# theopaid/Parallel-Image-Convolution-using-MPI-OPENMP-and-CUDA

Measured on AMD Instinct MI355X. Metric: Mpixels/sec (and wall-time) for 1920x2520 RGB, 40 reps at 1/2/4/8 MI355X, higher is better.
Workload: dtype fp32-exact (packed 16-bit integer, bit-identical to the reference float32)

## Files before the change

parallel-image-convolution-using-mpi-openmp-and-cuda_amd/csrc/include/pconv/engine.hpp:

```cpp
#pragma once

#include <hip/hip_runtime_api.h>

#include <functional>
#include <map>
#include <memory>
#include <tuple>
#include <vector>

#include "pconv/device.hpp"
#include "pconv/filter.hpp"
#include "pconv/image.hpp"
#include "pconv/kernels.hpp"
#include "pconv/partition.hpp"
#include "pconv/schedule.hpp"

namespace pconv {

class BandEngine;

class HaloTransport {
 public:
  virtual ~HaloTransport() = default;
  virtual void exchange(BandEngine& e, int64_t depth, hipStream_t stream) = 0;
  virtual const char* name() const = 0;
  virtual bool capturable() const { return false; }
};

struct EngineOptions {
  int device = 0;
  int halo_depth = 1;
  int fuse = 1;
  bool overlap = true;
  bool use_graph = false;
  bool capture_exchanges = false;
  KernelVariant variant = KernelVariant::Auto;
  Border border = Border::Zero;
  hipStream_t compute_stream = nullptr;
  hipStream_t comm_stream = nullptr;
  bool timing = true;
  bool kernel_copies = false;
  int stream_chunks = 0;
  std::vector<int> stream_weights;
  int64_t stream_min_bytes = int64_t(8) << 20;
  bool cu_mask_queues = true;
  bool head_on_slot_streams = true;
  bool head_alt_uploads = true;
  bool lazy_head = true;
};

struct RunStats {
  double loop_ms = 0;
  double wall_ms = 0;
  int launches = 0;
  int exchanges = 0;
  int64_t image_launches = 0;
};

class BandEngine {
 public:
  BandEngine(const ImageGeom& geom, const Band& band, const Filter& filter, const EngineOptions& opt);
  ~BandEngine();

  const ImageGeom& geom() const { return geom_; }
  const Band& band() const { return band_; }
  const Filter& filter() const { return filter_; }
  const FrameLayout& layout() const { return lay_; }
  const EngineOptions& options() const { return opt_; }
  static constexpr size_t kMaxCachedGraphs = 64;
  size_t cached_graphs() const { return graphs_.size() + step_graphs_.size(); }
  size_t cached_step_graphs() const { return step_graphs_.size(); }
  hipStream_t compute_stream() const { return cs_; }
  hipStream_t comm_stream() const { return ms_; }

  void set_transport(std::shared_ptr<HaloTransport> t) { transport_ = std::move(t); }

  uint8_t* src_frame() const { return frame_[cur_].data() + lay_.offset(0); }
  uint8_t* dst_frame() const { return frame_[cur_ ^ 1].data() + lay_.offset(0); }
  uint8_t* frame_at(int which) const { return frame_[which & 1].data() + lay_.offset(0); }
  uint8_t* frame_base(int which) const { return frame_[which & 1].data(); }
  int cur() const { return cur_; }
  void set_cur(int c) { cur_ = c & 1; }

  void upload_rows(const uint8_t* host, int64_t host_pitch, int64_t r_begin, int64_t r_end,
                   hipStream_t stream = nullptr);
  void upload_rows_device(const uint8_t* dev, int64_t dev_pitch, int64_t r_begin, int64_t r_end);
  void set_halo_valid(bool v) { halo_valid_ = v; }
  bool input_preloaded(int64_t in_r0, int64_t in_r1) const;
  void download_rows(uint8_t* host, int64_t host_pitch, int64_t r_begin, int64_t r_end,
                     hipStream_t stream = nullptr);
  void download_rows_device(uint8_t* dev, int64_t dev_pitch, int64_t r_begin, int64_t r_end);

  void wait_stream(hipStream_t s);
  void signal_stream(hipStream_t s);

  void exchange_now(hipStream_t stream = nullptr);
  bool has_transport() const { return transport_ != nullptr; }

  void run(int reps);
  uint64_t residual();
  StableStats run_until_stable(int max_reps, int check_every,
// ... 35 lines not shown
  DeviceBuffer frame_[2];
  int cur_ = 0;
  bool halo_valid_ = false;
  int pre_exchanges_ = 0;
  DeviceBuffer res_count_;
  PinnedBuffer res_host_;
  Event res_ev_;
  uint64_t res_seen_ = 0;
  Stream own_cs_, own_ms_;
  hipStream_t cs_ = nullptr, ms_ = nullptr;
  Event ev_ready_, ev_halo_, ev_t0_, ev_t1_, ev_sync_;
  std::vector<Event> up_evs_, dn_evs_;
  bool stream_trace_ = false;
  std::vector<Event> st_ev_;
  size_t st_chunks_ = 0;
 public:
  void set_stream_trace(bool on) { stream_trace_ = on; }
  std::vector<std::vector<double>> stream_trace();
  std::vector<double> time_residual(int launches);
  void reserve_stream_events(size_t chunks) {
    while (up_evs_.size() < chunks) up_evs_.push_back(Event::create());
    while (dn_evs_.size() < chunks + 1) dn_evs_.push_back(Event::create());
  }

 private:
  std::shared_ptr<HaloTransport> transport_;
  RunStats stats_;
  double wall_t0_ = 0;
  bool timing_pending_ = false;
  std::map<std::pair<int, int>, hipGraphExec_t> graphs_;
  struct StepGraph {
    hipGraphExec_t exec = nullptr;
    int end_cur = 0;
    int launches = 0;
    int exchanges = 0;
  };
  void trim_graph_caches();
  std::map<std::tuple<int, int, const uint8_t*, int64_t, int64_t, uint8_t*>, StepGraph> step_graphs_;
};

class BandPipeline {
 public:
  BandPipeline(const ImageGeom& geom, const Band& band, const Filter& filter, const EngineOptions& opt, int slots,
               int concurrent = -1, bool slot_streams = false, bool step_graphs = true, bool slot_comm = false);
  ~BandPipeline();
  int slots() const { return static_cast<int>(slots_.size()); }
  BandEngine& slot(int i) { return *slots_.at(i); }
  void set_transport(std::shared_ptr<HaloTransport> t);
  void set_slot_transport(int k, std::shared_ptr<HaloTransport> t);
  void submit(const uint8_t* host_in, int64_t in_r0, int64_t in_r1, uint8_t* host_out, int reps);
  void drain();
  int64_t submitted() const { return count_; }
  int64_t streamed_heads() const { return streamed_heads_; }
  bool concurrent() const { return concurrent_; }
  bool graphs() const { return graphs_; }
  bool step_graphs() const { return graphs_ && step_graphs_; }
  void enable_trace(int images);
  std::vector<std::vector<double>> trace();
  void enable_marks(int images);
  std::vector<std::vector<double>> marks();
  bool ready(int k);
  void wait_image(int k);

 private:
  void trace_mark(int stage, hipStream_t s);
  void completion_mark(int k, bool before, bool streamed);
  void submit_image(int k, const uint8_t* host_in, int64_t in_r0, int64_t in_r1, uint8_t* host_out, int reps);
  struct HeldImage {
    const uint8_t* in = nullptr;
    int64_t r0 = 0, r1 = 0;
    uint8_t* out = nullptr;
    int reps = 0;
    bool valid = false;
  };
  HeldImage held_;
  bool force_graph_ = false;
  void issue_held(bool streamed);
  Stream h2d_, d2h_, comm_;
  std::vector<Stream> computes_;
  std::vector<Stream> slot_comms_;
  bool concurrent_ = false;
  bool graphs_ = false;
  bool step_graphs_ = true;
  std::vector<std::unique_ptr<BandEngine>> slots_;
  std::vector<Event> ev_up_, ev_done_, ev_free_, ev_halo_;
  int64_t burst_pos_ = 0;
  int64_t streamed_heads_ = 0;
  bool head_streaming_ = false;
  bool head_on_slots_ = false;
  Event ev_head_, h2d_wait_;
  std::vector<bool> used_;
  int64_t count_ = 0;
  std::vector<Event> trace_ev_;
  std::vector<int> trace_slot_;
  int64_t trace_first_ = 0;
  std::vector<Event> done_;
  Event burst_start_;
  std::vector<Event> mark_ev_;
  std::vector<std::pair<int, bool>> mark_info_;
  int64_t mark_first_ = 0;
};

class LocalCluster {
 public:
  LocalCluster(const ImageGeom& geom, int bands, const Filter& filter, const EngineOptions& opt);
  int size() const { return static_cast<int>(engines_.size()); }
  BandEngine& engine(int i) { return *engines_.at(i); }
  void upload(const uint8_t* host, bool preload_halo);
  void run(int reps, bool device_async = false);
  void download(uint8_t* host);
  void synchronize();

 private:
  ImageGeom geom_;
  std::vector<std::unique_ptr<BandEngine>> engines_;
  std::vector<Event> ev_phase_;
};

class NullTransport : public HaloTransport {
 public:
  void exchange(BandEngine&, int64_t, hipStream_t) override {}
  const char* name() const override { return "null (timing only)"; }
  bool capturable() const override { return true; }
};

class LocalTransport : public HaloTransport {
 public:
  explicit LocalTransport(std::vector<BandEngine*> peers) : peers_(std::move(peers)) {}
  void exchange(BandEngine& e, int64_t depth, hipStream_t stream) override;
  const char* name() const override { return "local-d2d"; }
  bool capturable() const override { return false; }

 private:
  std::vector<BandEngine*> peers_;
};

}
// ... 1 lines not shown
```

parallel-image-convolution-using-mpi-openmp-and-cuda_amd/csrc/include/pconv/schedule.hpp:

```cpp
#pragma once

#include <cstdint>
#include <string>
#include <vector>

#include "pconv/partition.hpp"

namespace pconv {

struct LaunchSpec {
  int steps = 1;
  int64_t lo = 0, hi = 0;
  bool after_halo = false;
};

struct Phase {
  int64_t exchange_depth = 0;
  int steps = 1;
  std::vector<LaunchSpec> launches;
};

struct PlanConfig {
  int halo_depth = 1;
  int fuse = 1;
  bool overlap = true;
  bool halo_preloaded = false;
};

std::vector<Phase> plan_band(const Band& band, int reps, const PlanConfig& cfg);

std::string describe_plan(const std::vector<Phase>& plan);

struct StreamChunk {
  int64_t up_lo = 0, up_hi = 0;
  std::vector<LaunchSpec> launches;
  std::vector<int> levels;
  int64_t down_lo = 0, down_hi = 0;
};

struct StreamPlan {
  int levels = 0;
  std::vector<StreamChunk> chunks;
};

bool streamable(const std::vector<Phase>& plan);

std::vector<int64_t> stream_cuts(int64_t in_lo, int64_t in_hi, int chunks);
std::vector<int64_t> stream_cuts_weighted(int64_t in_lo, int64_t in_hi, const std::vector<int>& weights);

StreamPlan plan_streamed(const std::vector<Phase>& plan, int64_t in_lo, int64_t in_hi, int64_t owned_rows,
                         const std::vector<int64_t>& cuts);

PlanConfig normalize_plan_config(PlanConfig cfg, int64_t min_band_rows, int max_fuse);

}
```

parallel-image-convolution-using-mpi-openmp-and-cuda_amd/csrc/src/engine.cpp:

```cpp
#include "pconv/engine.hpp"

#include <cstring>

#include "pconv/trace.hpp"

#include <algorithm>
#include <atomic>
#include <cstdlib>
#include <thread>

namespace pconv {

namespace {

PlanConfig engine_plan_config(const ImageGeom& geom, const Band& band, const Filter& f, const EngineOptions& opt) {
  PlanConfig c;
  c.fuse = supports_fusion(f, opt.variant) ? opt.fuse : 1;
  c.halo_depth = opt.halo_depth;
  c.overlap = opt.overlap;
  const int64_t min_rows = band.world > 1 ? geom.height / band.world : 0;
  return normalize_plan_config(c, min_rows, kMaxFusedSteps);
}

}
// ... 616 lines not shown
    }
    if (step_graphs && opt.stream_chunks > 1) {
      head_on_slots_ = opt.head_on_slot_streams && slots >= 3;
      if (!head_on_slots_) {
        h2d_ = Stream::create(0);
        d2h_ = Stream::create(0);
      }
      ev_head_ = Event::create();
      h2d_wait_ = Event::create();
      head_streaming_ = true;
      const size_t nchunks = std::max(static_cast<size_t>(std::max(opt.stream_chunks, 0)), opt.stream_weights.size());
      for (auto& e : slots_) e->reserve_stream_events(nchunks + 1);
      const int64_t rb = slots_[0]->layout().row_bytes;
      PinnedBuffer row(static_cast<size_t>(rb));
      std::memset(row.data(), 0, row.size());
      for (auto& e : slots_) {
        e->upload_rows(row.data(), rb, 0, 1, e->compute_stream());
        e->download_rows(row.data(), rb, 0, 1, e->compute_stream());
      }
      for (auto& e : slots_) e->synchronize();
    }
    used_.assign(slots, false);
    for (int i = 0; i < slots; ++i) done_.push_back(Event::create(true));
    burst_start_ = Event::create(true);
    return;
  }
  const bool nb = band.up >= 0 || band.down >= 0;
  int hw_queues = 4;
  if (const char* q = std::getenv("GPU_MAX_HW_QUEUES")) hw_queues = std::max(1, std::atoi(q));
  const int fixed = 2 + (nb ? 1 : 0);
  concurrent_ = concurrent < 0 ? (slots > 1 && hw_queues >= fixed + slots) : (concurrent > 0 && slots > 1);
  h2d_ = Stream::create(0);
  d2h_ = Stream::create(0);
  EngineOptions o = opt;
  o.use_graph = false;
  o.timing = false;
  if (nb) {
    comm_ = Stream::create(-1);
    o.comm_stream = comm_.get();
  }
  for (int i = 0; i < (concurrent_ ? slots : 1); ++i) computes_.push_back(Stream::create(0));
  for (int i = 0; i < slots; ++i) {
    o.compute_stream = computes_[concurrent_ ? i : 0].get();
    slots_.push_back(std::make_unique<BandEngine>(geom, band, filter, o));
    ev_up_.push_back(Event::create());
    ev_done_.push_back(Event::create());
    ev_free_.push_back(Event::create());
    ev_halo_.push_back(Event::create());
  }
  used_.assign(slots, false);
}

BandPipeline::~BandPipeline() {
  if (h2d_.get()) (void)hipStreamSynchronize(h2d_.get());
  for (auto& c : computes_) (void)hipStreamSynchronize(c.get());
  for (auto& c : slot_comms_) (void)hipStreamSynchronize(c.get());
  if (d2h_.get()) (void)hipStreamSynchronize(d2h_.get());
  if (comm_.get()) (void)hipStreamSynchronize(comm_.get());
}

void BandPipeline::set_slot_transport(int k, std::shared_ptr<HaloTransport> t) {
  PCONV_CHECK(graphs_, "per-slot transports need the slot-stream pipeline");
  slots_.at(k)->set_transport(std::move(t));
}

void BandPipeline::set_transport(std::shared_ptr<HaloTransport> t) {
  for (auto& s : slots_) s->set_transport(t);
}

void BandPipeline::submit(const uint8_t* host_in, int64_t in_r0, int64_t in_r1, uint8_t* host_out, int reps) {
  TraceRange tr("pconv.pipeline.submit");
  if (held_.valid) issue_held(false);
  const int k = static_cast<int>(count_ % static_cast<int64_t>(slots_.size()));
  if (graphs_ && step_graphs_ && head_streaming_ && burst_pos_ == 0 && slots_[0]->options().lazy_head) {
    burst_start_.record(slots_[static_cast<size_t>(k)]->compute_stream());
    completion_mark(k, true, false);
    held_ = HeldImage{host_in, in_r0, in_r1, host_out, reps, true};
    return;
  }
  if (graphs_ && burst_pos_ == 0) burst_start_.record(slots_[static_cast<size_t>(k)]->compute_stream());
  completion_mark(k, true, false);
  const int64_t heads = streamed_heads_;
  submit_image(k, host_in, in_r0, in_r1, host_out, reps);
  completion_mark(k, false, streamed_heads_ != heads);
  if (graphs_) done_[static_cast<size_t>(k)].record(slots_[static_cast<size_t>(k)]->compute_stream());
}

void BandPipeline::issue_held(bool streamed) {
  const HeldImage h = held_;
  held_.valid = false;
  const int k = static_cast<int>(count_ % static_cast<int64_t>(slots_.size()));
  const int64_t heads = streamed_heads_;
  force_graph_ = !streamed;
  submit_image(k, h.in, h.r0, h.r1, h.out, h.reps);
  force_graph_ = false;
  completion_mark(k, false, streamed_heads_ != heads);
  done_[static_cast<size_t>(k)].record(slots_[static_cast<size_t>(k)]->compute_stream());
}

bool BandPipeline::ready(int k) {
  if (held_.valid) issue_held(true);
  const hipError_t e = hipEventQuery(done_.at(static_cast<size_t>(k)).get());
  if (e == hipErrorNotReady) return false;
  PCONV_HIP_CHECK(e);
  return true;
}

void BandPipeline::wait_image(int k) {
  if (held_.valid) issue_held(true);
  done_.at(static_cast<size_t>(k)).sync();
}

void BandPipeline::completion_mark(int k, bool before, bool streamed) {
  if (mark_ev_.empty()) return;
  const int64_t i = count_ - mark_first_ - (before ? 0 : 1);
  if (i < 0 || i + 1 >= static_cast<int64_t>(mark_ev_.size())) return;
  if (before && i != 0) return;
  hipStream_t s = graphs_ ? slots_[static_cast<size_t>(k)]->compute_stream() : (before ? h2d_.get() : d2h_.get());
  if (before) {
    mark_ev_[0].record(s);
    return;
  }
  mark_ev_[static_cast<size_t>(i + 1)].record(s);
  mark_info_.emplace_back(k, streamed);
}

void BandPipeline::enable_marks(int images) {
  PCONV_CHECK(images >= 0, "mark capacity must be >= 0");
  mark_ev_.clear();
  mark_info_.clear();
  if (images == 0) return;
  for (int i = 0; i <= images; ++i) mark_ev_.push_back(Event::create(true));
  mark_first_ = count_;
}

std::vector<std::vector<double>> BandPipeline::marks() {
  drain();
  std::vector<std::vector<double>> out;
  for (size_t i = 0; i < mark_info_.size(); ++i)
    out.push_back({static_cast<double>(mark_info_[i].first), Event::elapsed_ms(mark_ev_[0], mark_ev_[i + 1]),
                   mark_info_[i].second ? 1.0 : 0.0});
  mark_ev_.clear();
  mark_info_.clear();
  return out;
}

void BandPipeline::submit_image(int k, const uint8_t* host_in, int64_t in_r0, int64_t in_r1, uint8_t* host_out,
                                int reps) {
  BandEngine& e = *slots_[static_cast<size_t>(k)];
  if (graphs_ && !step_graphs_) {
    const bool preloaded = e.input_preloaded(in_r0, in_r1);
    hipStream_t cs = e.compute_stream();
    trace_mark(0, cs);
    e.upload_rows(host_in, e.layout().row_bytes, in_r0, in_r1);
    trace_mark(1, cs);
    if (!preloaded && e.exchange_free(reps, true)) {
      e.exchange_now(cs);
    } else {
      e.set_halo_valid(preloaded);
    }
    e.run(reps);
    trace_mark(2, cs);
    e.download_rows(host_out, e.layout().row_bytes, 0, e.band().rows);
    trace_mark(3, cs);
    used_[k] = true;
    ++count_;
    return;
  }
  if (graphs_) {
    PCONV_CHECK(trace_ev_.empty(), "pipeline trace needs directly issued images (graph capture off)");
    const int64_t in_bytes = (in_r1 - in_r0) * e.layout().row_bytes;
    if (burst_pos_ == 0 && head_streaming_ && !force_graph_ && in_bytes >= e.options().stream_min_bytes) {
      const StreamPlan sp = e.stream_plan(reps, in_r0, in_r1);
      if (!sp.chunks.empty()) {
        e.set_cur(0);
        const int n = slots();
        hipStream_t up = head_on_slots_ ? computes_[static_cast<size_t>((k + 1) % n)].get() : h2d_.get();
        hipStream_t down = head_on_slots_ ? computes_[static_cast<size_t>((k + n - 1) % n)].get() : d2h_.get();
        hipStream_t up2 = head_on_slots_ && n >= 4 && e.options().head_alt_uploads
                              ? computes_[static_cast<size_t>((k + 2) % n)].get()
                              : nullptr;
        h2d_wait_.record(e.compute_stream());
        h2d_wait_.wait_on(up);
        if (up2) h2d_wait_.wait_on(up2);
        hipStream_t done = e.enqueue_streamed(host_in, in_r0, in_r1, host_out, sp, up, down, up2);
        if (done != e.compute_stream()) {
          ev_head_.record(done);
          ev_head_.wait_on(e.compute_stream());
        }
        ++burst_pos_;
        used_[k] = true;
        ++count_;
        ++streamed_heads_;
        return;
      }
    }
    e.process_graph(host_in, in_r0, in_r1, host_out, reps);
    ++burst_pos_;
    used_[k] = true;
    ++count_;
    return;
  }
  const bool preloaded = e.input_preloaded(in_r0, in_r1);
  if (used_[k]) ev_free_[k].wait_on(h2d_.get());
  if (e.options().stream_chunks > 1 && trace_ev_.empty()) {
    const StreamPlan sp = e.stream_plan(reps, in_r0, in_r1);
    if (!sp.chunks.empty()) {
      hipStream_t done = e.enqueue_streamed(host_in, in_r0, in_r1, host_out, sp, h2d_.get(), d2h_.get());
      ev_free_[k].record(done);
      used_[k] = true;
      ++count_;
      return;
    }
  }
  trace_mark(0, h2d_.get());
  e.upload_rows(host_in, e.layout().row_bytes, in_r0, in_r1, h2d_.get());
  trace_mark(1, h2d_.get());
  ev_up_[k].record(h2d_.get());
  e.set_halo_valid(preloaded);
  if (!preloaded && comm_.get() && e.has_transport() && reps > 0) {
    ev_up_[k].wait_on(comm_.get());
    e.exchange_now(comm_.get());
    ev_halo_[k].record(comm_.get());
    ev_halo_[k].wait_on(e.compute_stream());
  } else {
// ... 139 lines not shown
```

parallel-image-convolution-using-mpi-openmp-and-cuda_amd/csrc/src/py_module.cpp:

```cpp
#include <omp.h>
#include <pybind11/pybind11.h>
#include <pybind11/stl.h>

#include <cstring>

#include "pconv/app.hpp"
#include "pconv/batch_engine.hpp"
#include "pconv/cpu_stencil.hpp"
#include "pconv/device.hpp"
#include "pconv/engine.hpp"
#include "pconv/ipc_halo.hpp"
#include "pconv/kernels.hpp"
#include "pconv/partition.hpp"
#include "pconv/selftest.hpp"
#include "pconv/raw_io.hpp"
#include "pconv/rccl_comm.hpp"
#include "pconv/schedule.hpp"
#include "../kernels/swar.hpp"

namespace py = pybind11;
using namespace pconv;

namespace {

// ... 94 lines not shown
      });
  m.def("row_band", &row_band, py::arg("height"), py::arg("world"), py::arg("rank"));
  m.def("row_bands", &row_bands, py::arg("height"), py::arg("world"));
  m.def("reference_rows_division", &reference_rows_division);

  py::class_<LaunchSpec>(m, "LaunchSpec")
      .def_readonly("steps", &LaunchSpec::steps)
      .def_readonly("lo", &LaunchSpec::lo)
      .def_readonly("hi", &LaunchSpec::hi)
      .def_readonly("after_halo", &LaunchSpec::after_halo);
  py::class_<Phase>(m, "Phase")
      .def_readonly("exchange_depth", &Phase::exchange_depth)
      .def_readonly("steps", &Phase::steps)
      .def_readonly("launches", &Phase::launches);
  m.def(
      "plan_band",
      [](const Band& b, int reps, int halo_depth, int fuse, bool overlap, bool halo_preloaded) {
        PlanConfig c;
        c.halo_depth = halo_depth;
        c.fuse = fuse;
        c.overlap = overlap;
        c.halo_preloaded = halo_preloaded;
        return plan_band(b, reps, c);
      },
      py::arg("band"), py::arg("reps"), py::arg("halo_depth") = 1, py::arg("fuse") = 1, py::arg("overlap") = true,
      py::arg("halo_preloaded") = false);
  m.def(
      "normalize_plan",
      [](int halo_depth, int fuse, int64_t min_band_rows, int max_fuse) {
        PlanConfig c;
        c.halo_depth = halo_depth;
        c.fuse = fuse;
        c = normalize_plan_config(c, min_band_rows, max_fuse);
        return py::make_tuple(c.halo_depth, c.fuse);
      },
      py::arg("halo_depth"), py::arg("fuse"), py::arg("min_band_rows"), py::arg("max_fuse") = kMaxFusedSteps);
  m.def("describe_plan", &describe_plan);
  m.attr("MAX_FUSED_STEPS") = kMaxFusedSteps;
  py::class_<StreamChunk>(m, "StreamChunk")
      .def_readonly("up_lo", &StreamChunk::up_lo)
      .def_readonly("up_hi", &StreamChunk::up_hi)
      .def_readonly("launches", &StreamChunk::launches)
      .def_readonly("levels", &StreamChunk::levels)
      .def_readonly("down_lo", &StreamChunk::down_lo)
      .def_readonly("down_hi", &StreamChunk::down_hi);
  py::class_<StreamPlan>(m, "StreamPlan")
      .def_readonly("levels", &StreamPlan::levels)
      .def_readonly("chunks", &StreamPlan::chunks);
  m.def("streamable", &streamable, py::arg("plan"));
  m.def("stream_cuts", &stream_cuts, py::arg("in_lo"), py::arg("in_hi"), py::arg("chunks"));
  m.def("stream_cuts_weighted", &stream_cuts_weighted, py::arg("in_lo"), py::arg("in_hi"), py::arg("weights"));
  m.def("plan_streamed", &plan_streamed, py::arg("plan"), py::arg("in_lo"), py::arg("in_hi"), py::arg("owned_rows"),
        py::arg("cuts"));

  m.def(
      "cpu_convolve",
      [](py::buffer in, py::buffer out, int64_t w, int64_t h, const std::string& ch, int reps, py::object filter,
         bool omp, int threads, const std::string& border) {
        const ImageGeom g = make_geom(w, h, ch);
        const Border bd = parse_border(border);
        const HostView a = host_view(in, false), b = host_view(out, true);
        PCONV_CHECK(a.size == g.bytes() && b.size == g.bytes(), "buffer size does not match the image geometry");
        const Filter f = make_filter(filter);
        py::gil_scoped_release nogil;
        cpu_convolve(f, g, a.ptr, b.ptr, reps, omp ? CpuBackend::OpenMP : CpuBackend::Serial, threads, bd);
      },
      py::arg("src"), py::arg("dst"), py::arg("width"), py::arg("height"), py::arg("channels"), py::arg("reps"),
      py::arg("filter") = "gaussian", py::arg("omp") = false, py::arg("threads") = 0, py::arg("border") = "zero");
  m.def("default_cpu_threads", &default_cpu_threads,
        "OpenMP team size used when none is set: affinity CPUs capped by the cgroup quota, minus one");
  m.def(
      "set_cpu_threads",
      [](int n) {
        omp_set_num_threads(std::max(1, n));
        return omp_get_max_threads();
      },
      py::arg("n"), "OpenMP team size of this process's CPU stencil (returns the size now in effect)");
  m.def("cpu_threads", []() { return omp_get_max_threads(); }, "OpenMP team size in effect");
  m.def("configure_cpu_threads", &configure_cpu_threads, py::arg("share") = 1,
        "Size the OpenMP team (unless OMP_NUM_THREADS is set) for `share` processes on this node");
  m.def(
      "cpu_fused_launch",
      [](py::object filter, const std::string& ch, int64_t row_bytes, int64_t rows, int64_t halo, py::buffer src,
         py::buffer dst, int64_t lo, int64_t hi, int steps, int64_t g_row0, int64_t height, bool omp,
         const std::string& border) {
        const Border bd = parse_border(border);
        const FrameLayout lay = FrameLayout::make(row_bytes, rows, halo);
        const HostView a = host_view(src, false), b = host_view(dst, true);
        PCONV_CHECK(a.size == lay.bytes() && b.size == lay.bytes(), "frame buffer size mismatch");
        const Filter f = make_filter(filter);
        py::gil_scoped_release nogil;
        cpu_fused_launch(f, parse_channels(ch), lay, a.ptr, b.ptr, lo, hi, steps, g_row0, height,
                         omp ? CpuBackend::OpenMP : CpuBackend::Serial, bd);
      },
      py::arg("filter"), py::arg("channels"), py::arg("row_bytes"), py::arg("rows"), py::arg("halo"), py::arg("src"),
      py::arg("dst"), py::arg("lo"), py::arg("hi"), py::arg("steps"), py::arg("g_row0"), py::arg("height"),
      py::arg("omp") = false, py::arg("border") = "zero");
  m.def(
      "cpu_residual",
      [](py::buffer in, int64_t w, int64_t h, const std::string& ch, py::object filter, bool omp, int threads,
         const std::string& border) {
        const ImageGeom g = make_geom(w, h, ch);
        const Border bd = parse_border(border);
        const HostView a = host_view(in, false);
        PCONV_CHECK(a.size == g.bytes(), "buffer size does not match the image geometry");
        const Filter f = make_filter(filter);
// ... 629 lines not shown
            e.upload_sized(reinterpret_cast<const uint8_t*>(ptr), to_sizes(sizes), device);
          },
          py::arg("ptr"), py::arg("sizes"), py::arg("device") = false)
      .def(
          "download_sized",
          [](BatchEngine& e, py::buffer host) {
            const HostView v = host_view(host, true);
            PCONV_CHECK(v.size >= packed_bytes(e.geom(), e.sizes()), "host buffer too small");
            e.download_sized(v.ptr);
          },
          py::arg("host"))
      .def(
          "download_sized_ptr",
          [](BatchEngine& e, uintptr_t ptr, bool device) { e.download_sized(reinterpret_cast<uint8_t*>(ptr), device); },
          py::arg("ptr"), py::arg("device") = false)
      .def_property_readonly("sizes",
                             [](const BatchEngine& e) {
                               std::vector<std::pair<int64_t, int64_t>> out;
                               for (const auto& z : e.sizes()) out.emplace_back(z.width, z.height);
                               return out;
                             })
      .def("wait_stream", [](BatchEngine& e, uintptr_t s) { e.wait_stream(reinterpret_cast<hipStream_t>(s)); })
      .def("signal_stream", [](BatchEngine& e, uintptr_t s) { e.signal_stream(reinterpret_cast<hipStream_t>(s)); })
      .def("run", &BatchEngine::run, py::arg("reps"), py::arg("n"), py::call_guard<py::gil_scoped_release>())
      .def("synchronize", &BatchEngine::synchronize, py::call_guard<py::gil_scoped_release>())
      .def("residual", &BatchEngine::residual, py::arg("n"), py::call_guard<py::gil_scoped_release>(),
           "per-image bytes of the newest frames of images [0, n) that one more repetition would change (one launch)")
      .def(
          "run_until_stable",
          [](BatchEngine& e, int max_reps, int check_every, int n, bool compact) {
            std::vector<StableStats> st;
            {
              py::gil_scoped_release nogil;
              st = e.run_until_stable(max_reps, check_every, n, compact);
            }
            py::list out;
            for (const auto& s : st) out.append(py::make_tuple(s.reps_done, s.converged, s.residual, s.checks));
            return out;
          },
          py::arg("max_reps"), py::arg("check_every"), py::arg("n"), py::arg("compact") = false,
          "[(reps_done, converged, residual, checks)] of images [0, n), each as a single-image run would report it; "
          "compact: converged images are retired from the launches that follow (same results, fewer image_launches)")
      .def("time_residual", &BatchEngine::time_residual, py::arg("launches"), py::arg("n"),
           py::call_guard<py::gil_scoped_release>(),
           "diagnostics: ms of each of `launches` residual launches over images [0, n) (stream events)")
      .def_property_readonly("stats", &BatchEngine::last_stats);

  py::class_<BandPipeline>(m, "BandPipeline")
      .def(py::init([](int64_t w, int64_t h, const std::string& ch, py::object filter, int rank, int world,
                       int device, int halo, int fuse, bool overlap, const std::string& variant, int slots,
                       int concurrent, bool graphs, bool step_graphs, py::object band, bool slot_comm,
                       int stream_chunks, bool cu_mask_queues, bool head_on_slot_streams,
                       int64_t stream_min_bytes, bool head_alt_uploads, std::vector<int> stream_weights,
                       bool lazy_head, const std::string& border) {
             EngineOptions o;
             o.border = parse_border(border);
             o.lazy_head = lazy_head;
             o.head_alt_uploads = head_alt_uploads;
             o.stream_chunks = stream_chunks;
             PCONV_CHECK(stream_weights.empty() || static_cast<int>(stream_weights.size()) == stream_chunks,
                         "stream_weights: one weight per chunk (stream_chunks of them)");
             o.stream_weights = std::move(stream_weights);
             o.stream_min_bytes = stream_min_bytes;
             o.cu_mask_queues = cu_mask_queues;
             o.head_on_slot_streams = head_on_slot_streams;
             o.device = device;
             o.halo_depth = halo;
             o.fuse = fuse;
             o.overlap = overlap;
             o.variant = parse_variant(variant);
             const ImageGeom g = make_geom(w, h, ch);
             const Band b = band.is_none() ? row_band(h, world, rank) : band.cast<Band>();
             return std::make_unique<BandPipeline>(g, b, make_filter(filter), o, slots, concurrent, graphs,
                                                   step_graphs, slot_comm);
           }),
           py::arg("width"), py::arg("height"), py::arg("channels"), py::arg("filter") = "gaussian",
           py::arg("rank") = 0, py::arg("world") = 1, py::arg("device") = 0, py::arg("halo") = 1, py::arg("fuse") = 1,
           py::arg("overlap") = true, py::arg("variant") = "auto", py::arg("slots") = 2, py::arg("concurrent") = -1,
           py::arg("graphs") = false, py::arg("step_graphs") = true,
           py::arg("band") = py::none(), py::arg("slot_comm") = false, py::arg("stream_chunks") = 0,
           py::arg("cu_mask_queues") = true, py::arg("head_on_slot_streams") = true,
           py::arg("stream_min_bytes") = EngineOptions{}.stream_min_bytes, py::arg("head_alt_uploads") = true,
           py::arg("stream_weights") = std::vector<int>{}, py::arg("lazy_head") = EngineOptions{}.lazy_head,
           py::arg("border") = "zero")
      .def_property_readonly("slots", &BandPipeline::slots)
      .def("slot", &BandPipeline::slot, py::return_value_policy::reference_internal)
      .def("attach_rccl",
           [](BandPipeline& p, std::shared_ptr<RcclComm> c) {
             p.set_transport(std::make_shared<RcclTransport>(std::move(c)));
           })
      .def("attach_transport", [](BandPipeline& p, std::shared_ptr<HaloTransport> t) { p.set_transport(std::move(t)); },
           py::keep_alive<1, 2>())
      .def("attach_slot_rccl",
           [](BandPipeline& p, int k, std::shared_ptr<RcclComm> c) {
             p.set_slot_transport(k, std::make_shared<RcclTransport>(std::move(c)));
           })
      .def("attach_slot_transport",
           [](BandPipeline& p, int k, std::shared_ptr<HaloTransport> t) { p.set_slot_transport(k, std::move(t)); },
           py::keep_alive<1, 3>())
      .def(
          "submit",
          [](BandPipeline& p, uintptr_t in_ptr, int64_t in_r0, int64_t in_r1, uintptr_t out_ptr, int reps) {
            py::gil_scoped_release nogil;
            p.submit(reinterpret_cast<const uint8_t*>(in_ptr), in_r0, in_r1, reinterpret_cast<uint8_t*>(out_ptr), reps);
          },
          py::arg("in_ptr"), py::arg("in_r0"), py::arg("in_r1"), py::arg("out_ptr"), py::arg("reps"))
      .def("drain", &BandPipeline::drain, py::call_guard<py::gil_scoped_release>())
      .def("ready", &BandPipeline::ready, py::arg("slot"), "slot-stream mode: the slot's latest image is done")
      .def("wait_image", &BandPipeline::wait_image, py::arg("slot"), py::call_guard<py::gil_scoped_release>(),
           "slot-stream mode: block until the slot's latest image is done")
      .def("enable_marks", &BandPipeline::enable_marks, py::arg("images"),
           "Completion marks of the next `images` submits (a diagnostic pass; see marks()).")
      .def("marks", &BandPipeline::marks, py::call_guard<py::gil_scoped_release>(),
           "Drain, then per marked image [slot, ms from the first image's issue to its completion, head-streamed].")
      .def_property_readonly("submitted", &BandPipeline::submitted)
      .def_property_readonly("concurrent", &BandPipeline::concurrent)
      .def_property_readonly("graphs", &BandPipeline::graphs)
      .def_property_readonly("streamed_heads", &BandPipeline::streamed_heads)
      .def_property_readonly("step_graphs", &BandPipeline::step_graphs)
      .def_property_readonly("options",
                             [](BandPipeline& p) {
                               const EngineOptions& o = p.slot(0).options();
                               py::dict d;
                               d["stream_chunks"] = o.stream_chunks;
                               d["stream_weights"] = o.stream_weights;
                               d["lazy_head"] = o.lazy_head;
                               d["stream_min_bytes"] = o.stream_min_bytes;
                               d["head_alt_uploads"] = o.head_alt_uploads;
                               d["cu_mask_queues"] = o.cu_mask_queues;
                               d["head_on_slot_streams"] = o.head_on_slot_streams;
                               return d;
                             })
      .def("enable_trace", &BandPipeline::enable_trace, py::arg("images"),
           "Time the stages of the next `images` submits (directly issued pipelines only)")
      .def("trace", &BandPipeline::trace, py::call_guard<py::gil_scoped_release>(),
           "Per traced image: [slot, H2D start, H2D end, reps end, D2H end] in ms");

  py::class_<LocalCluster>(m, "LocalCluster")
      .def(py::init([](int64_t w, int64_t h, const std::string& ch, py::object filter, int bands, int device, int halo,
                       int fuse, const std::string& variant, bool overlap, const std::string& border) {
             EngineOptions o;
             o.border = parse_border(border);
             o.device = device;
             o.halo_depth = halo;
             o.fuse = fuse;
             o.overlap = overlap;
             o.variant = parse_variant(variant);
             return std::make_unique<LocalCluster>(make_geom(w, h, ch), bands, make_filter(filter), o);
           }),
           py::arg("width"), py::arg("height"), py::arg("channels"), py::arg("filter") = "gaussian",
           py::arg("bands") = 2, py::arg("device") = 0, py::arg("halo") = 1, py::arg("fuse") = 1,
           py::arg("variant") = "auto", py::arg("overlap") = true, py::arg("border") = "zero")
      .def("upload",
           [](LocalCluster& c, py::buffer host, bool preload_halo) {
             c.upload(host_view(host, false).ptr, preload_halo);
           },
           py::arg("host"), py::arg("preload_halo") = false)
      .def("run", &LocalCluster::run, py::arg("reps"), py::arg("device_async") = false,
           py::call_guard<py::gil_scoped_release>(),
           "device_async: every band through the production phase path (comm stream || interior, event-ordered)")
      .def("download", [](LocalCluster& c, py::buffer host) { c.download(host_view(host, true).ptr); })
      .def("exchanges", [](LocalCluster& c) { return c.engine(0).last_stats().exchanges; })
      .def_property_readonly("size", &LocalCluster::size);

  m.def("ipc_create_segment", &ipc_create_segment, py::arg("name"), py::arg("world"), py::arg("slots"),
        "create the zeroed shared flag segment of an IPC halo job (one rank)");
  m.def("ipc_pull_probe", &ipc_pull_probe, py::arg("form"), py::arg("bytes"), py::arg("host_source"),
        py::arg("iters") = 50, py::arg("device") = 0, py::arg("workgroups") = 0,
        py::call_guard<py::gil_scoped_release>(),
        "ms per IPC exchange of one pull form (grid|single|sdma), `bytes` per side from a pinned host buffer "
        "(host_source: stand-in for a peer GPU behind xGMI) or this GPU's HBM; self-neighbour flag protocol");
  m.def("ipc_grid_workgroups", &ipc_grid_workgroups, py::arg("bytes"));
  m.def("ipc_unlink_segment", &ipc_unlink_segment, py::arg("name"),
        "remove the segment's name (mappings stay valid; call once every rank has mapped it)");
  py::class_<IpcHaloTransport, HaloTransport, std::shared_ptr<IpcHaloTransport>>(m, "IpcHaloTransport")
      .def(py::init([](BandEngine& e, const std::string& segment, int slot, int slots, double timeout_s,
                       const std::string& pull) {
             return std::make_shared<IpcHaloTransport>(e, segment, slot, slots, timeout_s, parse_ipc_pull(pull));
           }),
// ... 77 lines not shown
```

parallel-image-convolution-using-mpi-openmp-and-cuda_amd/csrc/src/schedule.cpp:

```cpp
#include "pconv/schedule.hpp"

#include <algorithm>
#include <sstream>

#include "pconv/common.hpp"

namespace pconv {

PlanConfig normalize_plan_config(PlanConfig cfg, int64_t min_band_rows, int max_fuse) {
  cfg.fuse = std::max(1, std::min(cfg.fuse, max_fuse));
  cfg.halo_depth = std::max(cfg.halo_depth, cfg.fuse);
  if (min_band_rows > 0 && cfg.halo_depth > min_band_rows)
    cfg.halo_depth = static_cast<int>(std::max<int64_t>(1, min_band_rows));
  cfg.fuse = std::min(cfg.fuse, cfg.halo_depth);
  return cfg;
}

std::vector<Phase> plan_band(const Band& band, int reps, const PlanConfig& cfg) {
  PCONV_CHECK(reps >= 0, "reps must be >= 0");
  PCONV_CHECK(cfg.fuse >= 1 && cfg.halo_depth >= cfg.fuse, "plan: need 1 <= fuse <= halo_depth");
  const bool has_up = band.up >= 0, has_down = band.down >= 0;
  const bool has_nb = has_up || has_down;
  const int64_t rows = band.rows;
  PCONV_CHECK(!has_nb || cfg.halo_depth <= rows, "plan: halo depth exceeds band rows");
// ... 68 lines not shown
StreamPlan plan_streamed(const std::vector<Phase>& plan, int64_t in_lo, int64_t in_hi, int64_t owned_rows,
                         const std::vector<int64_t>& cuts) {
  PCONV_CHECK(streamable(plan), "plan_streamed: the plan must be exchange-free with one launch per phase");
  PCONV_CHECK(in_lo <= 0 && in_hi >= owned_rows && in_lo < in_hi, "plan_streamed: input rows must cover the band");
  for (size_t i = 0; i < cuts.size(); ++i)
    PCONV_CHECK(cuts[i] > in_lo && cuts[i] < in_hi && (i == 0 || cuts[i] > cuts[i - 1]),
                "plan_streamed: cuts must increase strictly inside the input rows");
  const int L = static_cast<int>(plan.size());
  std::vector<int64_t> lo(L + 1), hi(L + 1);
  std::vector<int> s(L + 1, 0);
  lo[0] = in_lo;
  hi[0] = in_hi;
  for (int j = 1; j <= L; ++j) {
    const LaunchSpec& l = plan[j - 1].launches[0];
    lo[j] = l.lo;
    hi[j] = l.hi;
    s[j] = l.steps;
  }
  PCONV_CHECK(lo[L] <= 0 && hi[L] >= owned_rows, "plan_streamed: the last level must cover the owned rows");
  StreamPlan sp;
  sp.levels = L;
  std::vector<int64_t> front(lo);
  front[0] = in_lo;
  const size_t C = cuts.size() + 1;
  for (size_t c = 0; c < C; ++c) {
    const bool last = c + 1 == C;
    StreamChunk ch;
    ch.up_lo = front[0];
    ch.up_hi = last ? in_hi : cuts[c];
    std::vector<int64_t> w(L + 1);
    w[0] = ch.up_hi;
    for (int j = 1; j <= L; ++j) {
      int64_t wj;
      if (last || w[j - 1] >= hi[j - 1])
        wj = hi[j];
      else
        wj = std::min(hi[j], w[j - 1] - std::max(s[j], s[j - 1]));
      wj = std::max(wj, front[j]);
      w[j] = wj;
      if (wj > front[j]) {
        ch.launches.push_back({s[j], front[j], wj, false});
        ch.levels.push_back(j);
      }
    }
    ch.down_lo = std::max<int64_t>(0, front[L]);
    ch.down_hi = std::min(owned_rows, w[L]);
    if (ch.down_hi < ch.down_lo) ch.down_hi = ch.down_lo;
    for (int j = 0; j <= L; ++j) front[j] = w[j];
    sp.chunks.push_back(std::move(ch));
  }
  return sp;
}

std::string describe_plan(const std::vector<Phase>& plan) {
  std::ostringstream os;
  for (size_t i = 0; i < plan.size(); ++i) {
    const Phase& p = plan[i];
    os << "phase " << i << ": steps=" << p.steps;
    if (p.exchange_depth) os << " exchange=" << p.exchange_depth;
    for (const auto& l : p.launches)
      os << " [" << l.lo << "," << l.hi << ")" << (l.after_halo ? "*" : "");
    os << "\n";
  }
  return os.str();
}

}
```

parallel-image-convolution-using-mpi-openmp-and-cuda_amd/parallel/dist_engine.py:

```python
from __future__ import annotations

from typing import Optional, Sequence

import numpy as np

from .._native import require_native
from ..models.filters import get_filter
from .bootstrap import env_context, make_rccl_comm

AUTO_HALO_CAP = 64


def auto_halo(height: int, world: int, reps: Optional[int], fuse: int, preload: bool = False) -> int:
    if world <= 1:
        return fuse
    band = height // world
    if preload and reps and int(reps) <= band:
        return max(int(reps), fuse, 1)
    d = min(AUTO_HALO_CAP, band)
    if reps:
        d = min(d, int(reps))
    return max(d, fuse, 1)


def preload_is_exchange_free(height: int, world: int, reps: int) -> bool:
    return world <= 1 or int(reps) <= height // world


def pcie_bytes_per_image(width: int, height: int, channels: str, world: int, rank: int, halo: int,
                         preload: bool) -> tuple:
    rb = int(width) * {"grey": 1, "rgb": 3, "rgba": 4}[channels]
    base, rem = divmod(int(height), int(world))
    rows = base + (1 if rank < rem else 0)
    y0 = rank * base + min(rank, rem)
    above = min(int(halo), y0) if preload and world > 1 else 0
    below = min(int(halo), int(height) - (y0 + rows)) if preload and world > 1 else 0
    return (rows + above + below) * rb, rows * rb


class DistributedBlur:
    def __init__(self, width: int, height: int, channels: str = "grey", filter="gaussian",
                 reps: Optional[int] = None, *, rank: Optional[int] = None, world: Optional[int] = None,
                 device: Optional[int] = None, halo: Optional[int] = None, fuse: Optional[int] = None,
                 overlap: bool = True, preload_halo: bool = False, comm=None, slots: int = 2,
                 variant: str = "auto", graph: bool = False, transport: str = "rccl", concurrent: int = -1,
                 step_graphs: Optional[bool] = None, graph_capture: bool = True, slot_exchange: bool = False,
                 self_neighbours: bool = False, slot_comm: bool = False, stream_chunks: int = 0,
                 ipc_timeout_s: float = 30.0, ipc_pull: str = "grid", cu_mask_queues: bool = True,
                 head_on_slot_streams: bool = True, stream_min_bytes: Optional[int] = None,
                 head_alt_uploads: bool = True, qualify_staging: bool = True, flush_staging: bool = True,
                 stream_weights: Optional[Sequence[int]] = None, lazy_head: Optional[bool] = None,
                 border: str = "zero"):
        n = require_native()
        ctx = env_context()
        self.rank = ctx.rank if rank is None else int(rank)
        self.world = ctx.world if world is None else int(world)
        self.device = ctx.local_rank if device is None else int(device)
        self.width, self.height, self.channels = int(width), int(height), channels
        nf = get_filter(filter).to_native()
        if fuse is None:
            ch = {"grey": 1, "rgb": 3, "rgba": 4}[channels]
            fuse = n.auto_fuse(nf, variant, self.width * ch * (self.height // max(1, self.world)), ch)
        if halo is None:
            halo = auto_halo(self.height, self.world, reps, fuse, preload=bool(preload_halo) and not slot_exchange)
        if stream_weights:
            stream_chunks = len(stream_weights)
        self.border = border
        kw = dict(halo=int(halo), fuse=int(fuse), overlap=bool(overlap), variant=variant, slots=int(slots),
                  border=border,
                  concurrent=int(concurrent), stream_chunks=int(stream_chunks),
                  cu_mask_queues=bool(cu_mask_queues), head_on_slot_streams=bool(head_on_slot_streams),
                  head_alt_uploads=bool(head_alt_uploads),
                  stream_weights=[int(w) for w in (stream_weights or [])],
                  **({} if lazy_head is None else {"lazy_head": bool(lazy_head)}),
                  **({} if stream_min_bytes is None else {"stream_min_bytes": int(stream_min_bytes)}))
        if self_neighbours:
            b = n.row_band(self.height, self.world, self.rank)
            b.up = 0 if b.up >= 0 else -1
            b.down = 0 if b.down >= 0 else -1
            b.rank, b.world = 0, 1
            kw["band"] = b
        self.pipe = n.BandPipeline(self.width, self.height, channels, nf, self.rank, self.world, self.device, **kw)
        self.preload_halo = bool(preload_halo) and self.world > 1
        free = reps is not None and self.pipe.slot(0).exchange_free(int(reps), self.preload_halo)
        if self.world > 1 and transport == "none" and not free:
            raise ValueError(f"transport 'none' needs exchange-free images: {reps} reps with a "
                             f"{self.pipe.slot(0).halo}-row ghost zone (preload_halo={self.preload_halo}) exchange "
                             "halos; use transport rccl/gloo-host")
        if step_graphs and not free and not slot_exchange:
            raise ValueError("step_graphs needs exchange-free images (world 1, or preload_halo with halo >= reps)")
        self.slot_exchange = bool(slot_exchange) and self.world > 1
        if transport == "ipc" and self.world > 1 and not free and not self.slot_exchange:
            raise ValueError("transport 'ipc' exchanges per slot: use slot_exchange=True (one transport per slot)")
        if self.slot_exchange and transport not in ("rccl", "ipc"):
            graph_capture = False
        streamed = int(stream_chunks) > 1 and free and not self.slot_exchange and step_graphs is False
        if not streamed and (self.slot_exchange or (free if step_graphs is None else bool(step_graphs))):
            del self.pipe
            self.pipe = n.BandPipeline(self.width, self.height, channels, nf, self.rank, self.world, self.device,
                                       graphs=True, step_graphs=bool(graph_capture),
                                       slot_comm=bool(slot_comm) and self.slot_exchange, **kw)
        self.engine = self.pipe.slot(0)
        self.band = self.engine.band
        self.row_bytes = self.engine.row_bytes
        d = self.engine.halo
        b = self.band
        self.above = min(d, b.y0) if self.preload_halo else 0
        self.below = min(d, self.height - (b.y0 + b.rows)) if self.preload_halo else 0
        in_rows = b.rows + self.above + self.below
        self.slots = int(slots)
        self._in = [n.PinnedBuffer(in_rows * self.row_bytes) for _ in range(self.slots)]
        self._out = [n.PinnedBuffer(b.rows * self.row_bytes) for _ in range(self.slots)]
        self.staging = None
        if qualify_staging:
            self.staging = self._qualify_staging(in_rows)
        self.inputs = [np.asarray(x).reshape(in_rows, self.row_bytes) for x in self._in]
        self.outputs = [np.asarray(x).reshape(b.rows, self.row_bytes) for x in self._out]
        self.input, self.output = self.inputs[0], self.outputs[0]
        self.flush_staging = bool(flush_staging)
        self._next = 0
        self._pending = False
        self.comm = None
        self.transport = None
        self.slot_comms = []
        self.slot_transports = []
        self.ipc = []
        if self.slot_exchange and transport == "ipc":
# ... 147 lines not shown
```

Before: 624,700.

## Split lone images into row bands processed concurrently across slot streams

When a single held image is issued on its own (the streamed-head path), the image's band is now cut into one row piece per pipeline slot. Each piece gets a dedicated engine with a ghost zone as deep as the rep count and runs its own graph on that slot's compute stream, and the streams are joined back with events. The aim is to spread a lone image's upload, compute and download across several streams instead of serialising it on one slot. In exchange it recomputes the overlapping halo rows, keeps up to two cached sets of extra engines, and adds a trace facility.

Measured after the change: 614,500. -1.6%, worse.

```diff
diff --git a/parallel-image-convolution-using-mpi-openmp-and-cuda_amd/csrc/include/pconv/engine.hpp b/parallel-image-convolution-using-mpi-openmp-and-cuda_amd/csrc/include/pconv/engine.hpp
--- a/parallel-image-convolution-using-mpi-openmp-and-cuda_amd/csrc/include/pconv/engine.hpp
+++ b/parallel-image-convolution-using-mpi-openmp-and-cuda_amd/csrc/include/pconv/engine.hpp
@@ -47,6 +47,7 @@
   bool head_on_slot_streams = true;
   bool head_alt_uploads = true;
   bool lazy_head = true;
+  bool band_split = true;
 };
 
 struct RunStats {
@@ -188,6 +189,9 @@
   void drain();
   int64_t submitted() const { return count_; }
   int64_t streamed_heads() const { return streamed_heads_; }
+  int64_t split_images() const { return split_images_; }
+  void set_split_trace(bool on) { split_trace_ = on; }
+  std::vector<std::vector<double>> split_trace();
   bool concurrent() const { return concurrent_; }
   bool graphs() const { return graphs_; }
   bool step_graphs() const { return graphs_ && step_graphs_; }
@@ -211,7 +215,18 @@
   };
   HeldImage held_;
   bool force_graph_ = false;
+  bool single_ = false;
   void issue_held(bool streamed);
+  struct SplitSet {
+    int reps = 0;
+    int64_t r0 = 0, r1 = 0;
+    std::vector<SplitPiece> plan;
+    std::vector<std::unique_ptr<BandEngine>> eng;
+  };
+  static constexpr size_t kMaxSplitSets = 2;
+  static constexpr int64_t kSplitMaxBytes = int64_t(64) << 20;
+  SplitSet* split_set(int reps, int64_t in_r0, int64_t in_r1);
+  bool submit_split(int k, const uint8_t* host_in, int64_t in_r0, int64_t in_r1, uint8_t* host_out, int reps);
   Stream h2d_, d2h_, comm_;
   std::vector<Stream> computes_;
   std::vector<Stream> slot_comms_;
@@ -219,6 +234,12 @@
   bool graphs_ = false;
   bool step_graphs_ = true;
   std::vector<std::unique_ptr<BandEngine>> slots_;
+  std::vector<SplitSet> splits_;
+  std::vector<Event> split_join_;
+  int64_t split_images_ = 0;
+  bool split_trace_ = false;
+  std::vector<Event> split_tr_ev_;
+  size_t split_tr_bands_ = 0;
   std::vector<Event> ev_up_, ev_done_, ev_free_, ev_halo_;
   int64_t burst_pos_ = 0;
   int64_t streamed_heads_ = 0;
diff --git a/parallel-image-convolution-using-mpi-openmp-and-cuda_amd/csrc/include/pconv/schedule.hpp b/parallel-image-convolution-using-mpi-openmp-and-cuda_amd/csrc/include/pconv/schedule.hpp
--- a/parallel-image-convolution-using-mpi-openmp-and-cuda_amd/csrc/include/pconv/schedule.hpp
+++ b/parallel-image-convolution-using-mpi-openmp-and-cuda_amd/csrc/include/pconv/schedule.hpp
@@ -51,6 +51,16 @@
 StreamPlan plan_streamed(const std::vector<Phase>& plan, int64_t in_lo, int64_t in_hi, int64_t owned_rows,
                          const std::vector<int64_t>& cuts);
 
+struct SplitPiece {
+  int64_t own_lo = 0, own_hi = 0;
+  int64_t up_lo = 0, up_hi = 0;
+  int64_t y0 = 0;
+  bool up = false, down = false;
+};
+
+std::vector<SplitPiece> plan_split(int64_t rows, int64_t in_r0, int64_t in_r1, int64_t y0, int64_t height, int reps,
+                                   int pieces);
+
 PlanConfig normalize_plan_config(PlanConfig cfg, int64_t min_band_rows, int max_fuse);
 
 }
diff --git a/parallel-image-convolution-using-mpi-openmp-and-cuda_amd/csrc/src/engine.cpp b/parallel-image-convolution-using-mpi-openmp-and-cuda_amd/csrc/src/engine.cpp
--- a/parallel-image-convolution-using-mpi-openmp-and-cuda_amd/csrc/src/engine.cpp
+++ b/parallel-image-convolution-using-mpi-openmp-and-cuda_amd/csrc/src/engine.cpp
@@ -692,6 +692,13 @@
 }
 
 BandPipeline::~BandPipeline() {
+  if (held_.valid) {
+    try {
+      issue_held(true);
+    } catch (const std::exception&) {
+      held_.valid = false;
+    }
+  }
   if (h2d_.get()) (void)hipStreamSynchronize(h2d_.get());
   for (auto& c : computes_) (void)hipStreamSynchronize(c.get());
   for (auto& c : slot_comms_) (void)hipStreamSynchronize(c.get());
@@ -732,10 +739,92 @@
   const int k = static_cast<int>(count_ % static_cast<int64_t>(slots_.size()));
   const int64_t heads = streamed_heads_;
   force_graph_ = !streamed;
+  single_ = streamed;
   submit_image(k, h.in, h.r0, h.r1, h.out, h.reps);
   force_graph_ = false;
+  single_ = false;
   completion_mark(k, false, streamed_heads_ != heads);
   done_[static_cast<size_t>(k)].record(slots_[static_cast<size_t>(k)]->compute_stream());
+}
+
+BandPipeline::SplitSet* BandPipeline::split_set(int reps, int64_t in_r0, int64_t in_r1) {
+  for (auto& s : splits_)
+    if (s.reps == reps && s.r0 == in_r0 && s.r1 == in_r1) return &s;
+  const BandEngine& e = *slots_[0];
+  const Band& b = e.band();
+  SplitSet s;
+  s.reps = reps;
+  s.r0 = in_r0;
+  s.r1 = in_r1;
+  s.plan = plan_split(b.rows, in_r0, in_r1, b.y0, e.geom().height, reps, slots());
+  if (s.plan.empty()) return nullptr;
+  if (splits_.size() >= kMaxSplitSets) splits_.erase(splits_.begin());
+  EngineOptions o = e.options();
+  o.halo_depth = reps;
+  o.fuse = std::min(o.fuse, reps);
+  o.stream_chunks = 0;
+  o.stream_weights.clear();
+  for (size_t i = 0; i < s.plan.size(); ++i) {
+    const SplitPiece& p = s.plan[i];
+    Band pb;
+    pb.y0 = p.y0;
+    pb.rows = p.own_hi - p.own_lo;
+    pb.up = p.up ? 0 : -1;
+    pb.down = p.down ? 0 : -1;
+    o.compute_stream = computes_[i].get();
+    o.comm_stream = computes_[i].get();
+    s.eng.push_back(std::make_unique<BandEngine>(e.geom(), pb, e.filter(), o));
+  }
+  while (split_join_.size() < s.plan.size()) split_join_.push_back(Event::create());
+  splits_.push_back(std::move(s));
+  return &splits_.back();
+}
+
+bool BandPipeline::submit_split(int k, const uint8_t* host_in, int64_t in_r0, int64_t in_r1, uint8_t* host_out,
+                                int reps) {
+  BandEngine& e = *slots_[static_cast<size_t>(k)];
+  if (!e.options().band_split || slots() < 2 || reps < 1 || !host_out) return false;
+  if ((in_r1 - in_r0) * e.layout().row_bytes > kSplitMaxBytes) return false;
+  if (!e.exchange_free(reps, e.input_preloaded(in_r0, in_r1))) return false;
+  SplitSet* ss = split_set(reps, in_r0, in_r1);
+  if (!ss) return false;
+  TraceRange tr("pconv.split_image");
+  const int64_t rb = e.layout().row_bytes;
+  const size_t np = ss->plan.size();
+  const bool tr_on = split_trace_;
+  if (tr_on) {
+    while (split_tr_ev_.size() < 1 + np) split_tr_ev_.push_back(Event::create(true));
+    split_tr_bands_ = np;
+    split_tr_ev_[0].record(computes_[0].get());
+  }
+  hipStream_t sk = e.compute_stream();
+  for (size_t i = 0; i < np; ++i) {
+    const SplitPiece& p = ss->plan[i];
+    ss->eng[i]->process_graph(host_in + (p.up_lo - in_r0) * rb, p.up_lo - p.own_lo, p.up_hi - p.own_lo,
+                              host_out + p.own_lo * rb, reps);
+    if (tr_on) split_tr_ev_[1 + i].record(ss->eng[i]->compute_stream());
+  }
+  for (size_t i = 0; i < np; ++i) {
+    hipStream_t s = ss->eng[i]->compute_stream();
+    if (s == sk) continue;
+    split_join_[i].record(s);
+    split_join_[i].wait_on(sk);
+  }
+  ++burst_pos_;
+  used_[static_cast<size_t>(k)] = true;
+  ++count_;
+  ++streamed_heads_;
+  ++split_images_;
+  return true;
+}
+
+std::vector<std::vector<double>> BandPipeline::split_trace() {
+  std::vector<std::vector<double>> out;
+  if (!split_trace_ || split_tr_bands_ == 0) return out;
+  drain();
+  for (size_t i = 0; i < split_tr_bands_; ++i)
+    out.push_back({static_cast<double>(i), Event::elapsed_ms(split_tr_ev_[0], split_tr_ev_[1 + i])});
+  return out;
 }
 
 bool BandPipeline::ready(int k) {
@@ -811,6 +900,7 @@
     PCONV_CHECK(trace_ev_.empty(), "pipeline trace needs directly issued images (graph capture off)");
     const int64_t in_bytes = (in_r1 - in_r0) * e.layout().row_bytes;
     if (burst_pos_ == 0 && head_streaming_ && !force_graph_ && in_bytes >= e.options().stream_min_bytes) {
+      if (single_ && submit_split(k, host_in, in_r0, in_r1, host_out, reps)) return;
       const StreamPlan sp = e.stream_plan(reps, in_r0, in_r1);
       if (!sp.chunks.empty()) {
         e.set_cur(0);
diff --git a/parallel-image-convolution-using-mpi-openmp-and-cuda_amd/csrc/src/py_module.cpp b/parallel-image-convolution-using-mpi-openmp-and-cuda_amd/csrc/src/py_module.cpp
--- a/parallel-image-convolution-using-mpi-openmp-and-cuda_amd/csrc/src/py_module.cpp
+++ b/parallel-image-convolution-using-mpi-openmp-and-cuda_amd/csrc/src/py_module.cpp
@@ -170,6 +170,16 @@
   m.def("stream_cuts_weighted", &stream_cuts_weighted, py::arg("in_lo"), py::arg("in_hi"), py::arg("weights"));
   m.def("plan_streamed", &plan_streamed, py::arg("plan"), py::arg("in_lo"), py::arg("in_hi"), py::arg("owned_rows"),
         py::arg("cuts"));
+  py::class_<SplitPiece>(m, "SplitPiece")
+      .def_readonly("own_lo", &SplitPiece::own_lo)
+      .def_readonly("own_hi", &SplitPiece::own_hi)
+      .def_readonly("up_lo", &SplitPiece::up_lo)
+      .def_readonly("up_hi", &SplitPiece::up_hi)
+      .def_readonly("y0", &SplitPiece::y0)
+      .def_readonly("up", &SplitPiece::up)
+      .def_readonly("down", &SplitPiece::down);
+  m.def("plan_split", &plan_split, py::arg("rows"), py::arg("in_r0"), py::arg("in_r1"), py::arg("y0"),
+        py::arg("height"), py::arg("reps"), py::arg("pieces"));
 
   m.def(
       "cpu_convolve",
@@ -905,8 +915,9 @@
                        int concurrent, bool graphs, bool step_graphs, py::object band, bool slot_comm,
                        int stream_chunks, bool cu_mask_queues, bool head_on_slot_streams,
                        int64_t stream_min_bytes, bool head_alt_uploads, std::vector<int> stream_weights,
-                       bool lazy_head, const std::string& border) {
+                       bool lazy_head, const std::string& border, bool band_split) {
              EngineOptions o;
+             o.band_split = band_split;
              o.border = parse_border(border);
              o.lazy_head = lazy_head;
              o.head_alt_uploads = head_alt_uploads;
@@ -935,7 +946,7 @@
            py::arg("cu_mask_queues") = true, py::arg("head_on_slot_streams") = true,
            py::arg("stream_min_bytes") = EngineOptions{}.stream_min_bytes, py::arg("head_alt_uploads") = true,
            py::arg("stream_weights") = std::vector<int>{}, py::arg("lazy_head") = EngineOptions{}.lazy_head,
-           py::arg("border") = "zero")
+           py::arg("border") = "zero", py::arg("band_split") = EngineOptions{}.band_split)
       .def_property_readonly("slots", &BandPipeline::slots)
       .def("slot", &BandPipeline::slot, py::return_value_policy::reference_internal)
       .def("attach_rccl",
@@ -970,6 +981,10 @@
       .def_property_readonly("concurrent", &BandPipeline::concurrent)
       .def_property_readonly("graphs", &BandPipeline::graphs)
       .def_property_readonly("streamed_heads", &BandPipeline::streamed_heads)
+      .def_property_readonly("split_images", &BandPipeline::split_images)
+      .def("set_split_trace", &BandPipeline::set_split_trace, py::arg("on"))
+      .def("split_trace", &BandPipeline::split_trace, py::call_guard<py::gil_scoped_release>(),
+           "Drain, then per band of the latest split image: [band, band end] in ms")
       .def_property_readonly("step_graphs", &BandPipeline::step_graphs)
       .def_property_readonly("options",
                              [](BandPipeline& p) {
@@ -978,6 +993,7 @@
                                d["stream_chunks"] = o.stream_chunks;
                                d["stream_weights"] = o.stream_weights;
                                d["lazy_head"] = o.lazy_head;
+                               d["band_split"] = o.band_split;
                                d["stream_min_bytes"] = o.stream_min_bytes;
                                d["head_alt_uploads"] = o.head_alt_uploads;
                                d["cu_mask_queues"] = o.cu_mask_queues;
diff --git a/parallel-image-convolution-using-mpi-openmp-and-cuda_amd/csrc/src/schedule.cpp b/parallel-image-convolution-using-mpi-openmp-and-cuda_amd/csrc/src/schedule.cpp
--- a/parallel-image-convolution-using-mpi-openmp-and-cuda_amd/csrc/src/schedule.cpp
+++ b/parallel-image-convolution-using-mpi-openmp-and-cuda_amd/csrc/src/schedule.cpp
@@ -144,6 +144,32 @@
   return sp;
 }
 
+std::vector<SplitPiece> plan_split(int64_t rows, int64_t in_r0, int64_t in_r1, int64_t y0, int64_t height, int reps,
+                                   int pieces) {
+  PCONV_CHECK(rows >= 1 && y0 >= 0 && y0 + rows <= height, "plan_split: band outside image");
+  PCONV_CHECK(in_r0 <= 0 && in_r1 >= rows && y0 + in_r0 >= 0 && y0 + in_r1 <= height,
+              "plan_split: input rows must cover the band inside the image");
+  if (pieces < 2 || reps < 1 || rows < int64_t(pieces) * reps) return {};
+  const int64_t above = -in_r0, below = in_r1 - rows;
+  if ((y0 > 0 && above < reps) || (y0 + rows < height && below < reps)) return {};
+  std::vector<int64_t> cuts{0};
+  for (int i = 0; i < pieces; ++i) cuts.push_back(cuts.back() + rows / pieces + (i < rows % pieces ? 1 : 0));
+  std::vector<SplitPiece> out;
+  for (int i = 0; i < pieces; ++i) {
+    SplitPiece p;
+    p.own_lo = cuts[static_cast<size_t>(i)];
+    p.own_hi = cuts[static_cast<size_t>(i) + 1];
+    if (p.own_hi - p.own_lo < reps) return {};
+    p.up_lo = p.own_lo - std::min<int64_t>(reps, p.own_lo - in_r0);
+    p.up_hi = p.own_hi + std::min<int64_t>(reps, in_r1 - p.own_hi);
+    p.y0 = y0 + p.own_lo;
+    p.up = p.y0 > 0;
+    p.down = p.y0 + (p.own_hi - p.own_lo) < height;
+    out.push_back(p);
+  }
+  return out;
+}
+
 std::string describe_plan(const std::vector<Phase>& plan) {
   std::ostringstream os;
   for (size_t i = 0; i < plan.size(); ++i) {
diff --git a/parallel-image-convolution-using-mpi-openmp-and-cuda_amd/parallel/dist_engine.py b/parallel-image-convolution-using-mpi-openmp-and-cuda_amd/parallel/dist_engine.py
--- a/parallel-image-convolution-using-mpi-openmp-and-cuda_amd/parallel/dist_engine.py
+++ b/parallel-image-convolution-using-mpi-openmp-and-cuda_amd/parallel/dist_engine.py
@@ -50,7 +50,7 @@
                  head_on_slot_streams: bool = True, stream_min_bytes: Optional[int] = None,
                  head_alt_uploads: bool = True, qualify_staging: bool = True, flush_staging: bool = True,
                  stream_weights: Optional[Sequence[int]] = None, lazy_head: Optional[bool] = None,
-                 border: str = "zero"):
+                 border: str = "zero", band_split: Optional[bool] = None):
         n = require_native()
         ctx = env_context()
         self.rank = ctx.rank if rank is None else int(rank)
@@ -73,6 +73,7 @@
                   head_alt_uploads=bool(head_alt_uploads),
                   stream_weights=[int(w) for w in (stream_weights or [])],
                   **({} if lazy_head is None else {"lazy_head": bool(lazy_head)}),
+                  **({} if band_split is None else {"band_split": bool(band_split)}),
                   **({} if stream_min_bytes is None else {"stream_min_bytes": int(stream_min_bytes)}))
         if self_neighbours:
             b = n.row_band(self.height, self.world, self.rank)
```
